# mwhoffman/pygp

Measured on AMD Instinct MI355X. Metric: ExactGP log-lik+grad evals/sec at N=16384 D=8 SE-ARD fp64, higher is better.
Workload: dtype f64; 1 GPU; ExactGP SE-ARD fp64 loglik+grad, N=16384 D=8 (metric config); batched-theta path: 6 independent thetas per GPU per step through gpx_loglik_batch, X/y resident in HBM; safe_mode=False, safe_mode_switches=0, launch=one process, C ABI only (no torch)

## Files before the change

pygp_amd/csrc/gemm_f64.hip:

```cpp

#include "gpx_internal.h"

#include "gemm_tile.h"

template <int TA, int TB, typename G>
__global__ __launch_bounds__(G::NTH, G::MINW) void gemm_f64_kernel(GemmArgs g)
{
    constexpr int TILE = G::TILE, WTM = G::WTM, WTN = G::WTN;
    extern __shared__ __attribute__((aligned(16))) char smem_raw[];
    double *smem = reinterpret_cast<double *>(smem_raw);

    int tm = blockIdx.y, tn = blockIdx.x;
    if (g.tiles) {
        tm = g.tiles[2 * blockIdx.x];
        tn = g.tiles[2 * blockIdx.x + 1];
    } else {
        const int gx = gridDim.x, gy = gridDim.y;
        const int mgx = gx >> 3, mgy = gy >> 3;
        const bool macro = g.swizzle && !(gx & 7) && !(gy & 7) && !((mgx * mgy) & 7);
        const int lin = blockIdx.y * gx + blockIdx.x;
        int u = lin, ux = gx, uy = gy;
        int w = 0;
        if (macro) {
            const int xcd = lin & 7, q = lin >> 3;
            u = (q >> 6) * 8 + xcd;
            w = q & 63;
            ux = mgx;
            uy = mgy;
        }
        int um, un;
        if (g.order == 0) {
            um = u / ux; un = u - um * ux;
        } else if (g.order == 1) {
            um = u / ux; un = u - um * ux; um = uy - 1 - um;
        } else {
            un = u / uy; um = u - un * uy;
            if (g.order == 2) un = ux - 1 - un;
        }
        if (macro) {
            tm = um * 8 + (w >> 3);
            tn = un * 8 + (w & 7);
        } else {
            tm = um;
            tn = un;
        }
    }
    const int m0 = tm * TILE, n0 = tn * TILE;
    if ((g.flags & GEMM_UPPER_ONLY) && n0 + TILE <= m0) return;
    int klo = 0, khi = g.K;
    if (g.flags & GEMM_KLO_M) klo = max(klo, m0 - g.kshift);
    if (g.flags & GEMM_KHI_M) khi = min(khi, m0 + TILE);
    if (g.flags & GEMM_KLO_N) klo = max(klo, n0 - g.kshift);
    if (g.flags & GEMM_KHI_N) khi = min(khi, n0 + TILE);
    int zb = blockIdx.z, zm = 0;
    if (g.kchunk > 0) {
        if (g.nsplit > 0) {
            zm = zb / g.nsplit;
            zb -= zm * g.nsplit;
        }
        klo = max(klo, zb * g.kchunk);
        khi = min(khi, (zb + 1) * g.kchunk);
    }
    klo &= ~(BK - 1);

    const double *__restrict__ A = g.A + (long long)zb * g.strideA + (long long)zm * g.mstrideA;
    const double *__restrict__ B = g.B + (long long)zb * g.strideB + (long long)zm * g.mstrideB;
    double *__restrict__ C = g.C + (long long)zb * g.strideC + (long long)zm * g.mstrideC;

    const int tid = threadIdx.x;
    const int lane = tid & 63, wave = tid >> 6;
    const int wm = wave / G::WN, wn = wave % G::WN;
    const int lr = lane & 15, lk = lane >> 4;

    constexpr bool AKM = (TA == 1);
    constexpr bool BKM = (TB == 0);
    constexpr int AK = AKM ? 4 * G::KSTR : 4, AT = AKM ? 16 : 16 * MNSTR;
    constexpr int BKS = BKM ? 4 * G::KSTR : 4, BT = BKM ? 16 : 16 * MNSTR;

    const double alpha = g.alpha;
    const double beta = (g.beta0_from >= 0 && n0 >= g.beta0_from) ? 0.0 : g.beta;
    if (g.C2 && (m0 >> 7) != (n0 >> 7))
        C = g.C2 + (long long)zb * g.strideC2;
    v4d acc[WTM][WTN];
    if (beta != 0.0) {
        const double sc = beta / alpha;
#pragma unroll
        for (int i = 0; i < WTM; ++i)
#pragma unroll
            for (int j = 0; j < WTN; ++j) {
                const int col = n0 + wn * (TILE / G::WN) + j * 16 + lr;
#pragma unroll
                for (int r = 0; r < 4; ++r) {
                    const int row = m0 + wm * (TILE / G::WM) + i * 16 + lk + 4 * r;
                    acc[i][j][r] = sc * C[(size_t)row * g.ldc + col];
                }
            }
    } else {
#pragma unroll
        for (int i = 0; i < WTM; ++i)
#pragma unroll
            for (int j = 0; j < WTN; ++j) acc[i][j] = (v4d){0.0, 0.0, 0.0, 0.0};
    }

    const int nslice = (khi - klo) / BK;
    if (nslice > 0) {
        double *As = smem, *Bs = smem + 2 * G::OPER;
        const bool rev = (g.flags & GEMM_KREV) != 0;
        const int kfirst = rev ? khi - BK : klo, kstep = rev ? -BK : BK;
        const int amn = wm * (TILE / G::WM) + lr, bmn = wn * (TILE / G::WN) + lr;
        const double *ap0 = As + (AKM ? lk * G::KSTR + amn : amn * MNSTR + lk);
        const double *bp0 = Bs + (BKM ? lk * G::KSTR + bmn : bmn * MNSTR + lk);
        if constexpr (!G::DEEP) {
            Regs<G::NLOAD> ra, rb;
            ra = load_slice<G, AKM>(A, g.lda, m0, kfirst, tid);
            rb = load_slice<G, BKM>(B, g.ldb, n0, kfirst, tid);
            store_slice<G, AKM>(As, tid, ra);
            store_slice<G, BKM>(Bs, tid, rb);
            __syncthreads();
            for (int s = 0; s + 1 < nslice; ++s) {
                const int cur = s & 1;
                const int k0 = kfirst + (s + 1) * kstep;
                ra = load_slice<G, AKM>(A, g.lda, m0, k0, tid);
                rb = load_slice<G, BKM>(B, g.ldb, n0, k0, tid);
                mfma_slice<WTM, WTN, AK, AT, BKS, BT>(ap0 + cur * G::OPER,
                                                      bp0 + cur * G::OPER, acc);
                const int nxt = cur ^ 1;
                store_slice<G, AKM>(As + nxt * G::OPER, tid, ra);
                store_slice<G, BKM>(Bs + nxt * G::OPER, tid, rb);
                __syncthreads();
            }
            const int cur = (nslice - 1) & 1;
            mfma_slice<WTM, WTN, AK, AT, BKS, BT>(ap0 + cur * G::OPER, bp0 + cur * G::OPER,
                                                  acc);
        } else {
            Regs<G::NLOAD> ra0, rb0, ra1, rb1;
            const int last = nslice - 1;
            ra0 = load_slice<G, AKM>(A, g.lda, m0, kfirst, tid);
            rb0 = load_slice<G, BKM>(B, g.ldb, n0, kfirst, tid);
            {
                const int k1 = kfirst + min(1, last) * kstep;
                ra1 = load_slice<G, AKM>(A, g.lda, m0, k1, tid);
                rb1 = load_slice<G, BKM>(B, g.ldb, n0, k1, tid);
            }
            store_slice<G, AKM>(As, tid, ra0);
            store_slice<G, BKM>(Bs, tid, rb0);
            __syncthreads();
            for (int s = 0; s < nslice; s += 2) {
                {
                    const int k2 = kfirst + min(s + 2, last) * kstep;
                    ra0 = load_slice<G, AKM>(A, g.lda, m0, k2, tid);
                    rb0 = load_slice<G, BKM>(B, g.ldb, n0, k2, tid);
                    mfma_slice<WTM, WTN, AK, AT, BKS, BT>(ap0, bp0, acc);
                    store_slice<G, AKM>(As + G::OPER, tid, ra1);
                    store_slice<G, BKM>(Bs + G::OPER, tid, rb1);
                    __syncthreads();
                }
                {
                    const int k3 = kfirst + min(s + 3, last) * kstep;
                    ra1 = load_slice<G, AKM>(A, g.lda, m0, k3, tid);
                    rb1 = load_slice<G, BKM>(B, g.ldb, n0, k3, tid);
                    mfma_slice<WTM, WTN, AK, AT, BKS, BT>(ap0 + G::OPER, bp0 + G::OPER, acc);
                    store_slice<G, AKM>(As, tid, ra0);
                    store_slice<G, BKM>(Bs, tid, rb0);
                    __syncthreads();
                }
            }
        }
    }

#pragma unroll
    for (int i = 0; i < WTM; ++i)
#pragma unroll
        for (int j = 0; j < WTN; ++j)
#pragma unroll
            for (int r = 0; r < 4; ++r) {
                const int row = m0 + wm * (TILE / G::WM) + i * 16 + lk + 4 * r;
                const int col = n0 + wn * (TILE / G::WN) + j * 16 + lr;
                C[(size_t)row * g.ldc + col] = alpha * acc[i][j][r];
            }
}

typedef Geo<128, 2, 2> Big4;
typedef Geo<128, 2, 4> Big8;
typedef Geo<64, 2, 2> Small4;
typedef Geo<64, 2, 4> Small8;
typedef Geo<128, 2, 4, true> Big8D;
typedef Geo<64, 2, 4, true> Small8D;

#include <algorithm>
#include <atomic>
#include <cstdio>
#include <cstdlib>
#include <map>
#include <cstring>
#include <mutex>
#include <tuple>
#include <vector>

struct TileList {
    int *dev = nullptr;
    int count = 0;
};

#define GPX_MAX_DEVICES 64
static std::atomic<int> g_concurrent[GPX_MAX_DEVICES];
void gpx_gemm_concurrency(int device, int delta)
{
    if (device >= 0 && device < GPX_MAX_DEVICES) g_concurrent[device] += delta;
}
int gpx_gemm_concurrent(int device)
{
    return device >= 0 && device < GPX_MAX_DEVICES ? g_concurrent[device].load() : 0;
}

static int tile_order(int device)
{
    const int xcd_env = gpx_env().tile_xcd;
    return xcd_env >= 0 ? xcd_env : (gpx_gemm_concurrent(device) > 0 ? 0 : 1);
}

#define GEMM_SLOTS 512

static int tile_list(int device, int xcd_order, int tile, int Tm, int Tn, int K, int flags,
                     TileList *out, int part = 0, int slots = 0, int kshift = 0)
{
    typedef std::tuple<int, int, int, int, int, int, int, int> Key;
    static std::map<Key, TileList> cache;
    static std::mutex mu;
    const int sflags = flags & (GEMM_UPPER_ONLY | GEMM_KLO_M | GEMM_KHI_M | GEMM_KLO_N |
                                GEMM_KHI_N);
    const Key key(device, tile, Tm, Tn, K,
                  sflags | (xcd_order ? 1 << 20 : 0) | ((kshift / 64) << 5), part, slots);
    std::lock_guard<std::mutex> lock(mu);
    auto it = cache.find(key);
    if (it != cache.end()) {
        *out = it->second;
        return 0;
    }
    struct Item { int w, m, n; };
    std::vector<Item> items;
    items.reserve((size_t)Tm * Tn);
    const int gen_tile = part ? 128 : tile;
    for (int m = 0; m < Tm; ++m)
        for (int n = 0; n < Tn; ++n) {
            const int m0 = m * gen_tile, n0 = n * gen_tile;
            if ((sflags & GEMM_UPPER_ONLY) && n0 + gen_tile <= m0) continue;
            int klo = 0, khi = K;
            if (sflags & GEMM_KLO_M) klo = std::max(klo, m0 - kshift);
            if (sflags & GEMM_KHI_M) khi = std::min(khi, m0 + gen_tile);
            if (sflags & GEMM_KLO_N) klo = std::max(klo, n0 - kshift);
            if (sflags & GEMM_KHI_N) khi = std::min(khi, n0 + gen_tile);
            items.push_back({std::max(0, khi - klo), m, n});
        }
    if (xcd_order > 0 && items.size() >= 32 * 64) {
        const int MB = 8;
        const int Mm = (Tm + MB - 1) / MB, Mn = (Tn + MB - 1) / MB;
        struct Macro { long long w; std::vector<Item> t; };
        std::vector<Macro> macros((size_t)Mm * Mn);
        for (const Item &it : items) {
            Macro &mc = macros[(size_t)(it.m / MB) * Mn + it.n / MB];
            mc.w += it.w;
            mc.t.push_back(it);
        }
        std::vector<int> idx;
        for (size_t i = 0; i < macros.size(); ++i)
            if (!macros[i].t.empty()) idx.push_back((int)i);
        std::stable_sort(idx.begin(), idx.end(),
                         [&](int a, int b) { return macros[a].w > macros[b].w; });
        std::vector<Item> seq[8];
        long long load[8] = {0, 0, 0, 0, 0, 0, 0, 0};
        for (int id : idx) {
            int x = 0;
            for (int k = 1; k < 8; ++k)
                if (load[k] < load[x]) x = k;
            load[x] += macros[id].w;
            std::vector<Item> &t = macros[id].t;
            std::stable_sort(t.begin(), t.end(),
                             [](const Item &a, const Item &b) { return a.w > b.w; });
            seq[x].insert(seq[x].end(), t.begin(), t.end());
        }
        std::vector<Item> inter;
        inter.reserve(items.size());
        size_t pos[8] = {0, 0, 0, 0, 0, 0, 0, 0};
        while (inter.size() < items.size()) {
            for (int x = 0; x < 8; ++x) {
                if (pos[x] < seq[x].size()) {
                    inter.push_back(seq[x][pos[x]++]);
                } else {
                    int y = 0;
                    for (int k = 1; k < 8; ++k)
                        if (seq[k].size() - pos[k] > seq[y].size() - pos[y]) y = k;
                    if (pos[y] < seq[y].size()) inter.push_back(seq[y][pos[y]++]);
                }
            }
        }
        items.swap(inter);
    } else {
        std::stable_sort(items.begin(), items.end(),
                         [](const Item &a, const Item &b) { return a.w > b.w; });
    }
    if (part) {
        const size_t whole = slots > 0 ? items.size() / slots * slots : items.size();
        if (part == 1) {
            items.resize(whole);
        } else {
            std::vector<Item> rest;
            for (size_t i = whole; i < items.size(); ++i)
                for (int q = 0; q < 4; ++q) {
                    const int m = 2 * items[i].m + (q >> 1), n = 2 * items[i].n + (q & 1);
                    if ((sflags & GEMM_UPPER_ONLY) && n < m) continue;
                    rest.push_back({items[i].w, m, n});
                }
            items.swap(rest);
        }
    }
    std::vector<int> flat(items.size() * 2);
    for (size_t i = 0; i < items.size(); ++i) {
        flat[2 * i] = items[i].m;
        flat[2 * i + 1] = items[i].n;
    }
    TileList tl;
    tl.count = (int)items.size();
    if (tl.count > 0) {
        GPX_HIP(hipMalloc((void **)&tl.dev, flat.size() * sizeof(int)));
        GPX_HIP(hipMemcpy(tl.dev, flat.data(), flat.size() * sizeof(int),
                          hipMemcpyHostToDevice));
    GPX_HIP(hipDeviceSynchronize());
    }
    cache[key] = tl;
    *out = tl;
    return 0;
}

static void log_launch(hipStream_t s, int ta, int tb, int tile, const GemmArgs &g, int part,
                       int wgs)
{
    static FILE *f = nullptr;
    static bool init = false;
    static std::mutex mu;
    std::lock_guard<std::mutex> lock(mu);
    if (!init) {
        init = true;
        const char *e = gpx_env().gemm_log;
        if (e && *e) f = fopen(e, "w");
    }
    if (!f) return;
    fprintf(f, "%p %d %d %d %d %d %d %d %d %d %d %g\n", (void *)s, ta, tb, tile, g.M, g.N, g.K,
            g.flags, g.kshift, part, wgs, g.beta);
    fflush(f);
}

struct LaunchCtx {
    int device;
    int xcd_order;
};

template <int TA, int TB, typename G>
static int launch(hipStream_t s, const GemmArgs &g0, const LaunchCtx &lc, int part = 0)
{
    GemmArgs g = g0;
    const int structure = g.flags & (GEMM_UPPER_ONLY | GEMM_KLO_M | GEMM_KHI_M |
                                     GEMM_KLO_N | GEMM_KHI_N);
    g.tiles = nullptr;
    dim3 grid(g.N / G::TILE, g.M / G::TILE, g.batch > 0 ? g.batch : 1);
    if (part) {
        TileList tl;
        GPX_TRY(tile_list(lc.device, lc.xcd_order, G::TILE, g.M / 128, g.N / 128, g.K, g.flags,
                          &tl, part, GEMM_SLOTS));
        if (tl.count == 0) return 0;
        g.tiles = tl.dev;
        grid = dim3(tl.count, 1, 1);
    } else if (structure && g.use_lists) {
        TileList tl;
        GPX_TRY(tile_list(lc.device, lc.xcd_order, G::TILE, g.M / G::TILE, g.N / G::TILE, g.K,
                          g.flags, &tl, 0, 0, g.kshift));
        if (tl.count == 0) return 0;
        g.tiles = tl.dev;
        grid = dim3(tl.count, 1, g.batch > 0 ? g.batch : 1);
    }
    log_launch(s, TA, TB, G::TILE, g, part, (int)(grid.x * grid.y * grid.z));
    hipLaunchKernelGGL((gemm_f64_kernel<TA, TB, G>), grid, dim3(G::NTH), G::LDS_BYTES, s,
                       g);
    GPX_HIP(hipGetLastError());
    return 0;
}

template <int TA, int TB, typename G>
static int set_attr()
{
    GPX_HIP(hipFuncSetAttribute(reinterpret_cast<const void *>(&gemm_f64_kernel<TA, TB, G>),
                                hipFuncAttributeMaxDynamicSharedMemorySize, G::LDS_BYTES));
    return 0;
}

template <typename G>
static int set_attr_all()
{
    GPX_TRY((set_attr<0, 0, G>()));
    GPX_TRY((set_attr<0, 1, G>()));
    GPX_TRY((set_attr<1, 0, G>()));
    GPX_TRY((set_attr<1, 1, G>()));
    return 0;
}

int gpx_gemm_init()
{
    GPX_TRY(set_attr_all<Big4>());
    GPX_TRY(set_attr_all<Big8>());
    GPX_TRY(set_attr_all<Small4>());
    GPX_TRY(set_attr_all<Small8>());
    GPX_TRY(set_attr_all<Big8D>());
    GPX_TRY(set_attr_all<Small8D>());
    return 0;
}

template <typename G>
static int dispatch(hipStream_t s, int ta, int tb, const GemmArgs &g, const LaunchCtx &lc,
                    int part = 0)
{
    if (ta == 0 && tb == 0) return launch<0, 0, G>(s, g, lc, part);
    if (ta == 0 && tb == 1) return launch<0, 1, G>(s, g, lc, part);
    if (ta == 1 && tb == 0) return launch<1, 0, G>(s, g, lc, part);
    return launch<1, 1, G>(s, g, lc, part);
}

__global__ void gpx_jitter_kernel(long long ticks)
{
    const long long t0 = wall_clock64();
    while (wall_clock64() - t0 < ticks) __builtin_amdgcn_s_sleep(32);
}

int gpx_test_jitter(hipStream_t s)
{
    if (!gpx_env().test_jitter) return 0;
    static std::mutex mu;
    static unsigned long long state = 0;
    const int max_us = gpx_env().test_jitter_max_us;
    std::lock_guard<std::mutex> lock(mu);
    if (state == 0) state = 0x9E3779B97F4A7C15ull ^ (unsigned long long)gpx_env().test_jitter_seed;
    state = state * 6364136223846793005ull + 1442695040888963407ull;
    const unsigned r = (unsigned)(state >> 33);
    if (r & 1) return 0;
    const long long ticks = (long long)((r >> 1) % (unsigned)(max_us + 1)) * 100;
    hipLaunchKernelGGL(gpx_jitter_kernel, dim3(1), dim3(64), 0, s, ticks);
    GPX_HIP(hipGetLastError());
    return 0;
}

int gpx_gemm(hipStream_t s, int ta, int tb, const GemmArgs &g)
{
    if (g.M <= 0 || g.N <= 0) return 0;
    if (g.M % GPX_TILE || g.N % GPX_TILE || g.K % (2 * BK) || g.lda % 2 || g.ldb % 2) {
        gpx_set_error("gpx_gemm: unpadded operands M=%d N=%d K=%d lda=%d ldb=%d", g.M,
                      g.N, g.K, g.lda, g.ldb);
        return -1;
    }
    if (g.alpha == 0.0 && g.beta != 0.0) {
        gpx_set_error("gpx_gemm: alpha == 0 with beta = %g is not supported", g.beta);
        return -1;
    }
    if (((g.flags & (GEMM_KLO_M | GEMM_KLO_N)) && g.kshift % (2 * BK)) ||
        (g.kchunk > 0 && g.kchunk % (2 * BK))) {
        gpx_set_error("gpx_gemm: kshift=%d / kchunk=%d must be multiples of %d", g.kshift,
                      g.kchunk, 2 * BK);
        return -1;
    }
    GPX_TRY(gpx_test_jitter(s));
    LaunchCtx lc;
    GPX_HIP(hipGetDevice(&lc.device));
    lc.xcd_order = tile_order(lc.device);
    long long tiles = (long long)(g.M / 128) * (g.N / 128) * (g.batch > 0 ? g.batch : 1);
    if (g.flags & GEMM_UPPER_ONLY) tiles = tiles / 2 + g.M / 256;
    const int big_cfg = gpx_env().gemm_big;
    const int small_cfg = gpx_env().gemm_small;
    const int small_below = gpx_env().gemm_small_below;
    const int threshold = small_below > 0 ? small_below : 400;
    int tile = g.tile;
    if (tile == 0) tile = tiles < threshold ? 64 : 128;
    const int balance_on = gpx_env().gemm_nobalance ? 0 : 1;
    const int kstruct_ = g.flags & (GEMM_KLO_M | GEMM_KHI_M | GEMM_KLO_N | GEMM_KHI_N);
    if (balance_on && g.tile == 0 && tile == 128 && kstruct_ && g.use_lists && g.batch <= 1 &&
        g.kchunk == 0) {
        long long work = 0, longest = 0;
        for (int m0 = 0; m0 < g.M; m0 += 128)
            for (int n0 = 0; n0 < g.N; n0 += 128) {
                if ((g.flags & GEMM_UPPER_ONLY) && n0 + 128 <= m0) continue;
                int klo = 0, khi = g.K;
                if (g.flags & GEMM_KLO_M) klo = std::max(klo, m0 - g.kshift);
                if (g.flags & GEMM_KHI_M) khi = std::min(khi, m0 + 128);
                if (g.flags & GEMM_KLO_N) klo = std::max(klo, n0 - g.kshift);
                if (g.flags & GEMM_KHI_N) khi = std::min(khi, n0 + 128);
                const long long len = std::max(0, khi - klo);
                work += len;
                longest = std::max(longest, len);
            }
        const double S = GEMM_SLOTS;
        const double t128 = std::max((double)longest, work / S);
        const double t64 = std::max(longest / 4.0, 1.08 * work / S);
        if (t64 < 0.9 * t128) tile = 64;
    }
    const int split_on = gpx_env().gemm_nosplit ? 0 : 1;
    const int kstruct = g.flags & (GEMM_KLO_M | GEMM_KHI_M | GEMM_KLO_N | GEMM_KHI_N);
    if (split_on && !g.overlap && g.tile == 0 && tile == 128 && !kstruct && g.use_lists &&
        g.batch <= 1 && g.kchunk == 0 && !g.waves && !big_cfg && !small_cfg) {
        const long long S = GEMM_SLOTS;
        long long L = (long long)(g.M / 128) * (g.N / 128);
        if (g.flags & GEMM_UPPER_ONLY) {
            L = 0;
            for (int m = 0; m < g.M / 128; ++m) L += std::max(0, g.N / 128 - m);
        }
        const long long rem = L % S;
        if (L > S && rem != 0) {
            const double plain = (double)((L + S - 1) / S);
            const double split = (double)(L / S) + (double)((4 * rem + S - 1) / S) / 4.0 + 0.03;
            if (split < plain) {
                GPX_TRY(dispatch<Big8D>(s, ta, tb, g, lc, 1));
                return dispatch<Small8D>(s, ta, tb, g, lc, 2);
            }
        }
    }
    if (tile == 64) {
        const int sw = g.waves ? g.waves : small_cfg;
        if (sw == 4) return dispatch<Small4>(s, ta, tb, g, lc);
        if (sw == 8) return dispatch<Small8>(s, ta, tb, g, lc);
        return dispatch<Small8D>(s, ta, tb, g, lc);
    }
    const int bw = g.waves ? g.waves : big_cfg;
    const bool use4 = bw == 4;
    if (use4) return dispatch<Big4>(s, ta, tb, g, lc);
    if (bw == 8) return dispatch<Big8>(s, ta, tb, g, lc);
    return dispatch<Big8D>(s, ta, tb, g, lc);
}
```

pygp_amd/csrc/gpx_env.h:

```cpp
#pragma once

#include <cstdlib>
#include <cstring>
#include <vector>

#define GPX_ENV_TABLE(X)                                                        \
        \
    X(int, nb0, "GPX_NB0", 0)                                                   \
    X(int, nb, "GPX_NB", 0)                                                     \
    X(const char *, blocks_text, "GPX_BLOCKS", nullptr)                         \
    X(int, split_last, "GPX_SPLIT_LAST", 0)                                     \
    X(int, lookahead, "GPX_LOOKAHEAD", 1)                                       \
    X(int, fastchain, "GPX_FASTCHAIN", 1)                                       \
    X(int, aux, "GPX_AUX", 1)                                                   \
    X(int, lead_build, "GPX_LEAD_BUILD", 1)                                     \
    X(int, defer_kinv, "GPX_DEFER_KINV", 1)                                     \
    X(int, invcol_early, "GPX_INVCOL_EARLY", -1)                                \
    X(int, overlap_nosplit, "GPX_OVERLAP_NOSPLIT", 1)                           \
    X(int, grad_whole, "GPX_GRAD_WHOLE", 4096)                                  \
    X(int, grad_full_w, "GPX_GRAD_FULL_W", 4096)                                \
       \
    X(int, swizzle, "GPX_SWIZZLE", 0)                                           \
    X(int, tile_lists, "GPX_TILE_LISTS", 1)                                     \
    X(int, ord_t, "GPX_ORD_T", 2)                                               \
    X(int, ord_r12, "GPX_ORD_R12", 1)                                           \
    X(int, ord_lauum, "GPX_ORD_LAUUM", 0)                                       \
    X(int, krev, "GPX_KREV", 0)                                                 \
    X(int, krev_invcol, "GPX_KREV_INVCOL", 0)                                   \
    X(int, tile_xcd, "GPX_TILE_XCD", -1)                                        \
    X(int, gemm_big, "GPX_GEMM_BIG", 0)                                         \
    X(int, gemm_small, "GPX_GEMM_SMALL", 0)                                     \
    X(int, gemm_small_below, "GPX_GEMM_SMALL_BELOW", 0)                         \
    X(int, gemm_nobalance, "GPX_GEMM_NOBALANCE", 0)                             \
    X(int, gemm_nosplit, "GPX_GEMM_NOSPLIT", 0)                                 \
    X(const char *, gemm_log, "GPX_GEMM_LOG", nullptr)                          \
    X(int, ldpad, "GPX_LDPAD", 32)                                              \
    X(int, bench_ldpad, "GPX_BENCH_LDPAD", 0)                                   \
                                           \
    X(int, panel, "GPX_PANEL", -1)                                              \
    X(int, panel_stream, "GPX_PANEL_STREAM", 1)                                 \
    X(int, panel_serial, "GPX_PANEL_SERIAL", 1)                                 \
    X(int, panel_strict, "GPX_PANEL_STRICT", 0)                                 \
    X(int, panel_debug, "GPX_PANEL_DEBUG", 0)                                   \
    X(int, panel_timeout_ms, "GPX_PANEL_TIMEOUT_MS", 2000)                      \
    X(int, panel_timeout_us, "GPX_PANEL_TIMEOUT_US", 0)                         \
    X(int, panel_wg, "GPX_PANEL_WG", -1)                                        \
    X(int, panel_wg_wide, "GPX_PANEL_WG_WIDE", -1)                              \
    X(int, panel_wg_whole, "GPX_PANEL_WG_WHOLE", -1)                            \
    X(int, panel_nspine, "GPX_PANEL_NSPINE", -1)                                \
    X(int, panel_mspine, "GPX_PANEL_MSPINE", -1)                                \
    X(int, panel_mwg, "GPX_PANEL_MWG", -1)                                      \
    X(int, panel_split, "GPX_PANEL_SPLIT", 1)                                   \
    X(int, panel_fold, "GPX_PANEL_FOLD", 1)                                     \
    X(int, panel_kbatch, "GPX_PANEL_KBATCH", -1)                                \
    X(int, panel_i128, "GPX_PANEL_I128", -1)                                    \
    X(int, panel_u128, "GPX_PANEL_U128", 6)                                     \
    X(double, panel_chain_scale, "GPX_PANEL_CHAIN_SCALE", 0.75)                 \
    X(int, panel_whole, "GPX_PANEL_WHOLE", GPX_PANEL_WHOLE_DEFAULT)             \
    X(int, panel_rhs, "GPX_PANEL_RHS", 1)                                       \
    X(int, panel_wide, "GPX_PANEL_WIDE", 0)                                     \
    X(int, panel_leaf_skip, "GPX_PANEL_LEAF_SKIP", 0)                           \
    X(int, leaf_skip, "GPX_LEAF_SKIP", 0)                                       \
    X(int, leaf_mfma, "GPX_LEAF_MFMA", 1)                                       \
     \
    X(int, group_max_np, "GPX_GROUP_MAX_NP", 32768)                             \
    X(int, group_members, "GPX_GROUP_MEMBERS", 0)                               \
    X(int, group_inflight, "GPX_GROUP_INFLIGHT", 0)                             \
    X(int, group_min_big, "GPX_GROUP_MIN_BIG", 2)                               \
    X(int, sweep_min_members, "GPX_SWEEP_MIN_MEMBERS", 16)                      \
    X(int, sweep_lite, "GPX_SWEEP_LITE", 1)                                     \
    X(int, sweep_fold, "GPX_SWEEP_FOLD", -1)                                    \
    X(int, sweep_pre, "GPX_SWEEP_PRE", 1)                                       \
    X(int, sweep_right, "GPX_SWEEP_RIGHT", 4)                                   \
    X(int, sweep_invblock, "GPX_SWEEP_INVBLOCK", 4)                             \
    X(int, sweep_narrow, "GPX_SWEEP_NARROW", 1)                                 \
    X(int, sweep_rhs_dense, "GPX_SWEEP_RHS_DENSE", 1)                           \
    X(int, solo_max_np, "GPX_SOLO_MAX_NP", 0)                                   \
    X(int, solo_min_members, "GPX_SOLO_MIN_MEMBERS", 16)                        \
    X(int, xs_debug, "GPX_XS_DEBUG", 0)                                         \
     \
    X(int, batch_inflight, "GPX_BATCH_INFLIGHT", 3)                             \
    X(int, batch_lookahead, "GPX_BATCH_LOOKAHEAD", -1)                          \
    X(int, twin_probe, "GPX_TWIN_PROBE", 1)                                     \
    X(int, twin_own_bulk, "GPX_TWIN_OWN_BULK", 1)                               \
    X(bool, twin_log, "GPX_TWIN_LOG", false)                                    \
    X(bool, destroy_log, "GPX_DESTROY_LOG", false)                              \
    X(int, multi_fake, "GPX_MULTI_FAKE", 0)                                     \
    X(int, multi_force_rccl, "GPX_MULTI_FORCE_RCCL", 0)                         \
                                          \
    X(int, kbuild_w, "GPX_KBUILD_W", 0)                                         \
    X(int, trace_rows, "GPX_TRACE_ROWS", 16)                                    \
                                                                \
    X(const char *, test_jitter_text, "GPX_TEST_JITTER", nullptr)               \
    X(int, test_hold_build_us, "GPX_TEST_HOLD_BUILD_US", 0)

struct GpxEnv {
#define GPX_ENV_FIELD(type, field, name, dflt) type field;
    GPX_ENV_TABLE(GPX_ENV_FIELD)
#undef GPX_ENV_FIELD
    std::vector<int> blocks;
    bool test_jitter;
    long long test_jitter_seed;
    int test_jitter_max_us;

    static int read(const char *e, int dflt) { return e ? atoi(e) : dflt; }
    static double read(const char *e, double dflt) { return e ? atof(e) : dflt; }
    static bool read(const char *e, bool) { return e != nullptr; }
    static const char *read(const char *e, const char *) { return e; }

    GpxEnv()
    {
#define GPX_ENV_READ(type, field, name, dflt) field = read(getenv(name), (type)(dflt));
        GPX_ENV_TABLE(GPX_ENV_READ)
#undef GPX_ENV_READ
        auto within = [](int &v, int lo, int hi, int other) {
            if (v < lo || v > hi) v = other;
        };
        if (panel > 0 && (panel < 256 || panel > GPX_PANEL_MAX || panel % 128)) panel = GPX_PANEL_MAX;
        panel_whole = panel_whole < 0 ? 0 : (panel_whole > GPX_PANEL_WHOLE_MAX ? GPX_PANEL_WHOLE_MAX : panel_whole);
        panel_kbatch = panel_kbatch < 1 ? -1 : (panel_kbatch > 16 ? 16 : panel_kbatch);
        if (panel_timeout_ms < 1) panel_timeout_ms = 2000;
        within(panel_wg, 1, 256, -1);
        within(panel_wg_wide, 1, 96, -1);
        within(panel_wg_whole, 1, 250, -1);
        within(panel_nspine, 1, 8, -1);
        within(panel_mspine, 1, 9, -1);
        within(panel_mwg, 8, 1024, -1);
        within(group_inflight, 1, 4, 0);
        within(batch_inflight, 1, 8, 3);
        if (group_members > 256) group_members = 256;
        if (group_min_big < 2) group_min_big = 2;
        if (group_max_np < 0) group_max_np = 0;
        sweep_invblock = sweep_invblock < 1 ? 1 : (sweep_invblock > 8 ? 8 : sweep_invblock);
        if (ldpad < 0 || ldpad % 2) ldpad = 32;
        if (bench_ldpad < 0 || bench_ldpad % 2) bench_ldpad = 0;
        for (const char *e = blocks_text; e && *e;) {
            const int v = atoi(e);
            if (v >= GPX_TILE && v % GPX_TILE == 0) blocks.push_back(v);
            e = strchr(e, ',');
            if (e) ++e;
        }
        test_jitter = test_jitter_text != nullptr;
        test_jitter_seed = test_jitter ? atoll(test_jitter_text) : 0;
        const char *colon = test_jitter ? strchr(test_jitter_text, ':') : nullptr;
        test_jitter_max_us = colon ? atoi(colon + 1) : 300;
    }
};

inline const GpxEnv &gpx_env()
{
    static const GpxEnv env;
    return env;
}
```

Baseline: 14.81 evals/s.

## Add software-pipelined LDS-to-register MFMA loop to f64 GEMM kernel

Adds a PIPE template variant of the f64 GEMM kernel that prefetches the next k-step's A/B fragments from LDS into registers while MFMAs for the current step run, with scheduling barriers to keep the interleave. Global loads use precomputed per-thread byte offsets instead of recomputing addresses each slice. It also overlaps LDS stores of the next slice with the tail MFMAs before the barrier. The variant is on by default except for short-K 128-tile launches, and it raises register pressure, which may reduce occupancy.

```diff
diff --git a/pygp_amd/csrc/gemm_f64.hip b/pygp_amd/csrc/gemm_f64.hip
--- a/pygp_amd/csrc/gemm_f64.hip
+++ b/pygp_amd/csrc/gemm_f64.hip
@@ -3,7 +3,98 @@
 
 #include "gemm_tile.h"
 
-template <int TA, int TB, typename G>
+template <typename G, bool KMAJOR>
+__device__ __forceinline__ void slice_offsets(int ld, int tid, unsigned (&off)[G::NLOAD])
+{
+#pragma unroll
+    for (int c = 0; c < G::NLOAD; ++c) {
+        const int idx = tid + G::NTH * c;
+        if (KMAJOR) {
+            const int row = idx / (G::TILE / 2), c2 = idx % (G::TILE / 2);
+            off[c] = ((unsigned)row * (unsigned)ld + 2u * c2) * 8u;
+        } else {
+            const int row = idx >> 3, k2 = idx & 7;
+            off[c] = ((unsigned)row * (unsigned)ld + 2u * k2) * 8u;
+        }
+    }
+}
+
+template <bool KMAJOR>
+__device__ __forceinline__ const double *slice_base(const double *__restrict__ P, int ld, int mn0,
+                                                    int k0)
+{
+    return KMAJOR ? P + ((long long)k0 * ld + mn0) : P + ((long long)mn0 * ld + k0);
+}
+
+template <typename G>
+__device__ __forceinline__ Regs<G::NLOAD> load_slice_at(const double *base,
+                                                        unsigned (&off)[G::NLOAD])
+{
+    Regs<G::NLOAD> out;
+#pragma unroll
+    for (int c = 0; c < G::NLOAD; ++c) {
+        asm volatile("" : "+v"(off[c]));
+        out.v[c] = *reinterpret_cast<const double2 *>(reinterpret_cast<const char *>(base) +
+                                                      (size_t)off[c]);
+    }
+    return out;
+}
+
+template <int WTM, int WTN, int AT, int BT>
+__device__ __forceinline__ void pipe_read(const double *__restrict__ ap,
+                                          const double *__restrict__ bp, double (&a)[WTM],
+                                          double (&b)[WTN])
+{
+#pragma unroll
+    for (int t = 0; t < WTN; ++t) b[t] = bp[t * BT];
+#pragma unroll
+    for (int t = 0; t < WTM; ++t) a[t] = ap[t * AT];
+}
+
+#define PIPE_FENCE() __builtin_amdgcn_sched_barrier(0x2 | 0x4)
+
+template <int WTM, int WTN, int AT, int BT, bool READ_NEXT = true>
+__device__ __forceinline__ void pipe_step(const double *__restrict__ apn,
+                                          const double *__restrict__ bpn, double (&a)[WTM],
+                                          double (&b)[WTN], v4d (&acc)[WTM][WTN])
+{
+    static_assert(WTM % 2 == 0, "rows are taken in pairs");
+    constexpr bool INPLACE = WTM >= 4;
+    double an[WTM], bn[WTN];
+    if (READ_NEXT) {
+#pragma unroll
+        for (int t = 0; t < WTN; ++t) bn[t] = bpn[t * BT];
+        if (!INPLACE) {
+#pragma unroll
+            for (int t = 0; t < WTM; ++t) an[t] = apn[t * AT];
+        }
+    }
+    PIPE_FENCE();
+#pragma unroll
+    for (int i = 0; i < WTM; i += 2) {
+#pragma unroll
+        for (int r = i; r < i + 2; ++r)
+#pragma unroll
+            for (int j = 0; j < WTN; ++j)
+                acc[r][j] = __builtin_amdgcn_mfma_f64_16x16x4f64(a[r], b[j], acc[r][j], 0, 0, 0);
+        PIPE_FENCE();
+        if (READ_NEXT && INPLACE) {
+            a[i] = apn[i * AT];
+            a[i + 1] = apn[(i + 1) * AT];
+            PIPE_FENCE();
+        }
+    }
+    if (READ_NEXT) {
+#pragma unroll
+        for (int t = 0; t < WTN; ++t) b[t] = bn[t];
+        if (!INPLACE) {
+#pragma unroll
+            for (int t = 0; t < WTM; ++t) a[t] = an[t];
+        }
+    }
+}
+
+template <int TA, int TB, typename G, int PIPE>
 __global__ __launch_bounds__(G::NTH, G::MINW) void gemm_f64_kernel(GemmArgs g)
 {
     constexpr int TILE = G::TILE, WTM = G::WTM, WTN = G::WTN;
@@ -110,7 +201,83 @@
         const int amn = wm * (TILE / G::WM) + lr, bmn = wn * (TILE / G::WN) + lr;
         const double *ap0 = As + (AKM ? lk * G::KSTR + amn : amn * MNSTR + lk);
         const double *bp0 = Bs + (BKM ? lk * G::KSTR + bmn : bmn * MNSTR + lk);
-        if constexpr (!G::DEEP) {
+        if constexpr (PIPE) {
+            unsigned aoff[G::NLOAD], boff[G::NLOAD];
+            slice_offsets<G, AKM>(g.lda, tid, aoff);
+            slice_offsets<G, BKM>(g.ldb, tid, boff);
+            const int last = nslice - 1;
+            auto a_at = [&](int s) {
+                return load_slice_at<G>(slice_base<AKM>(A, g.lda, m0, kfirst + s * kstep), aoff);
+            };
+            auto b_at = [&](int s) {
+                return load_slice_at<G>(slice_base<BKM>(B, g.ldb, n0, kfirst + s * kstep), boff);
+            };
+            const double *ap1 = ap0 + G::OPER, *bp1 = bp0 + G::OPER;
+            double fa[WTM], fb[WTN];
+            if constexpr (!G::DEEP) {
+                Regs<G::NLOAD> ra = a_at(0), rb = b_at(0);
+                store_slice<G, AKM>(As, tid, ra);
+                store_slice<G, BKM>(Bs, tid, rb);
+                __syncthreads();
+                pipe_read<WTM, WTN, AT, BT>(ap0, bp0, fa, fb);
+                for (int s = 0; s < last; ++s) {
+                    const double *ap = (s & 1) ? ap1 : ap0, *bp = (s & 1) ? bp1 : bp0;
+                    const double *apx = (s & 1) ? ap0 : ap1, *bpx = (s & 1) ? bp0 : bp1;
+                    ra = a_at(s + 1);
+                    rb = b_at(s + 1);
+#pragma unroll
+                    for (int ks = 1; ks < BK / 4; ++ks)
+                        pipe_step<WTM, WTN, AT, BT>(ap + ks * AK, bp + ks * BKS, fa, fb, acc);
+                    const int nxt = (s & 1) ^ 1;
+                    store_slice<G, AKM>(As + nxt * G::OPER, tid, ra);
+                    store_slice<G, BKM>(Bs + nxt * G::OPER, tid, rb);
+                    __syncthreads();
+                    pipe_step<WTM, WTN, AT, BT>(apx, bpx, fa, fb, acc);
+                }
+                const double *ap = (last & 1) ? ap1 : ap0, *bp = (last & 1) ? bp1 : bp0;
+#pragma unroll
+                for (int ks = 1; ks < BK / 4; ++ks)
+                    pipe_step<WTM, WTN, AT, BT>(ap + ks * AK, bp + ks * BKS, fa, fb, acc);
+                pipe_step<WTM, WTN, AT, BT, false>(ap, bp, fa, fb, acc);
+            } else {
+                Regs<G::NLOAD> ra0 = a_at(0), rb0 = b_at(0);
+                Regs<G::NLOAD> ra1 = a_at(min(1, last)), rb1 = b_at(min(1, last));
+                store_slice<G, AKM>(As, tid, ra0);
+                store_slice<G, BKM>(Bs, tid, rb0);
+                __syncthreads();
+                pipe_read<WTM, WTN, AT, BT>(ap0, bp0, fa, fb);
+                for (int s = 0; s < nslice; s += 2) {
+                    {
+                        ra0 = a_at(min(s + 2, last));
+                        rb0 = b_at(min(s + 2, last));
+#pragma unroll
+                        for (int ks = 1; ks < BK / 4 - 1; ++ks)
+                            pipe_step<WTM, WTN, AT, BT>(ap0 + ks * AK, bp0 + ks * BKS, fa, fb,
+                                                        acc);
+                        store_slice<G, AKM>(As + G::OPER, tid, ra1);
+                        store_slice<G, BKM>(Bs + G::OPER, tid, rb1);
+                        pipe_step<WTM, WTN, AT, BT>(ap0 + (BK / 4 - 1) * AK,
+                                                    bp0 + (BK / 4 - 1) * BKS, fa, fb, acc);
+                        __syncthreads();
+                        pipe_step<WTM, WTN, AT, BT>(ap1, bp1, fa, fb, acc);
+                    }
+                    {
+                        ra1 = a_at(min(s + 3, last));
+                        rb1 = b_at(min(s + 3, last));
+#pragma unroll
+                        for (int ks = 1; ks < BK / 4 - 1; ++ks)
+                            pipe_step<WTM, WTN, AT, BT>(ap1 + ks * AK, bp1 + ks * BKS, fa, fb,
+                                                        acc);
+                        store_slice<G, AKM>(As, tid, ra0);
+                        store_slice<G, BKM>(Bs, tid, rb0);
+                        pipe_step<WTM, WTN, AT, BT>(ap1 + (BK / 4 - 1) * AK,
+                                                    bp1 + (BK / 4 - 1) * BKS, fa, fb, acc);
+                        __syncthreads();
+                        pipe_step<WTM, WTN, AT, BT>(ap0, bp0, fa, fb, acc);
+                    }
+                }
+            }
+        } else if constexpr (!G::DEEP) {
             Regs<G::NLOAD> ra, rb;
             ra = load_slice<G, AKM>(A, g.lda, m0, kfirst, tid);
             rb = load_slice<G, BKM>(B, g.ldb, n0, kfirst, tid);
@@ -379,8 +546,13 @@
         grid = dim3(tl.count, 1, g.batch > 0 ? g.batch : 1);
     }
     log_launch(s, TA, TB, G::TILE, g, part, (int)(grid.x * grid.y * grid.z));
-    hipLaunchKernelGGL((gemm_f64_kernel<TA, TB, G>), grid, dim3(G::NTH), G::LDS_BYTES, s,
-                       g);
+    const bool short_k = G::TILE == 128 && g.tile == 0 && g.waves == 0 && g.K <= 512;
+    if (gpx_env().gemm_pipe && !short_k)
+        hipLaunchKernelGGL((gemm_f64_kernel<TA, TB, G, 1>), grid, dim3(G::NTH), G::LDS_BYTES, s,
+                           g);
+    else
+        hipLaunchKernelGGL((gemm_f64_kernel<TA, TB, G, 0>), grid, dim3(G::NTH), G::LDS_BYTES, s,
+                           g);
     GPX_HIP(hipGetLastError());
     return 0;
 }
@@ -388,7 +560,9 @@
 template <int TA, int TB, typename G>
 static int set_attr()
 {
-    GPX_HIP(hipFuncSetAttribute(reinterpret_cast<const void *>(&gemm_f64_kernel<TA, TB, G>),
+    GPX_HIP(hipFuncSetAttribute(reinterpret_cast<const void *>(&gemm_f64_kernel<TA, TB, G, 0>),
+                                hipFuncAttributeMaxDynamicSharedMemorySize, G::LDS_BYTES));
+    GPX_HIP(hipFuncSetAttribute(reinterpret_cast<const void *>(&gemm_f64_kernel<TA, TB, G, 1>),
                                 hipFuncAttributeMaxDynamicSharedMemorySize, G::LDS_BYTES));
     return 0;
 }
diff --git a/pygp_amd/csrc/gpx_env.h b/pygp_amd/csrc/gpx_env.h
--- a/pygp_amd/csrc/gpx_env.h
+++ b/pygp_amd/csrc/gpx_env.h
@@ -33,6 +33,7 @@
     X(int, gemm_small_below, "GPX_GEMM_SMALL_BELOW", 0)                         \
     X(int, gemm_nobalance, "GPX_GEMM_NOBALANCE", 0)                             \
     X(int, gemm_nosplit, "GPX_GEMM_NOSPLIT", 0)                                 \
+    X(int, gemm_pipe, "GPX_GEMM_PIPE", 1)                                       \
     X(const char *, gemm_log, "GPX_GEMM_LOG", nullptr)                          \
     X(int, ldpad, "GPX_LDPAD", 32)                                              \
     X(int, bench_ldpad, "GPX_BENCH_LDPAD", 0)                                   \
```

Result: faster. 15.38 evals/s, median of 6 (+3.8%).
